# bwittmann/transoar

Measured on AMD Instinct MI355X. Metric: training-step CT volumes/s, 160x160x256 Focused-Decoder, higher is better.
Workload: dtype bf16

## Files before the change

### include/transoar_convgemm.h

```cpp
#ifndef TRANSOAR_CONVGEMM_H
#define TRANSOAR_CONVGEMM_H

#ifdef __cplusplus
extern "C" {
#endif

enum {
  TRANSOAR_CONVGEMM_OK = 0,
  TRANSOAR_CONVGEMM_ERR_NULL = -1,
  TRANSOAR_CONVGEMM_ERR_DIM = -2
};

int transoar_conv3d_igemm(const void* x, const void* wk, const float* bias, void* y, float* y32,
                          int N, int SD, int SH, int SW, int Cin, int Cout,
                          int MD, int MH, int MW, int src_stride,
                          int OD, int OH, int OW, int out_stride, int opd, int oph, int opw,
                          unsigned taps_d, unsigned taps_h, unsigned taps_w, int split, int classes, void* hip_stream);

int transoar_conv3d_finish(const float* y32, const float* bias, void* y, long rows, int cout, int split, void* hip_stream);

int transoar_conv3d_dgrad_s2_halo(const void* dy, const void* wkt, void* dx, int N, int OD, int OH, int OW, int D, int H, int W,
                                  int Cin, int Cout, void* hip_stream);

long transoar_conv3d_wgrad_part_floats(int Cin, int Cout, int chunks, int taps_out);
int transoar_conv3d_wgrad(const void* dy, const void* x, float* part, float* dw, int N, int SD, int SH, int SW, int Cin,
                          int Cout, int MD, int MH, int MW, int src_stride,
                          unsigned taps_d, unsigned taps_h, unsigned taps_w, int chunks, int taps_out, void* hip_stream);

int transoar_linear_wgrad_bias(const void* dy, const void* x, float* part, float* dw, float* bias_part, float* db, int T, int Cin,
                               int Cout, int chunks, void* hip_stream);

int transoar_conv3d_wgrad_ring(const void* dy, const void* x, float* part, float* dw, int N, int SD, int SH, int SW, int Cin,
                               int Cout, int MD, int MH, int MW, int src_stride, int chunks, void* hip_stream);

int transoar_conv3d_pack(const float* w, void* wk, void* wkt, int Cout, int Cin, void* hip_stream);

int transoar_conv3d_pack_many(const void* table, int n_layers, long total_tiles, void* hip_stream);

int transoar_convgemm_abi_version(void);

#ifdef __cplusplus
}
#endif
#endif
```

### transoar_amd/conv_gemm.py

```python
import os

import torch

from . import _native
from ._native import launch, ptr

ABI_VERSION = 3
CL3D = torch.channels_last_3d
lib = _native.bind("convgemm", abi=ABI_VERSION)


def _taps(entries):
    v = len(entries)
    for e, (delta, t) in enumerate(entries):
        v |= ((delta + 1) << (2 + 4 * e)) | (t << (4 + 4 * e))
    return v


TAPS_FWD = _taps([(-1, 0), (0, 1), (1, 2)])
TAPS_DGRAD1 = _taps([(1, 0), (0, 1), (-1, 2)])
TAPS_PARITY = (_taps([(0, 1)]), _taps([(1, 0), (0, 2)]))
TAPS_ONE = _taps([(0, 1)])

SPLIT_BELOW_TILES = 384
DGRAD_S2_HALO = os.environ.get("TRANSOAR_DGRAD_S2_HALO", "1") != "0"
WGRAD_BLOCKS = 512


def pack_fwd(weight):
    co, ci = weight.shape[:2]
    return weight.permute(2, 3, 4, 0, 1).reshape(27, co, ci).to(torch.bfloat16).contiguous()


def pack_dgrad(weight):
    co, ci = weight.shape[:2]
    return weight.permute(2, 3, 4, 1, 0).reshape(27, ci, co).to(torch.bfloat16).contiguous()


def pack_both(weight):
    co, ci = weight.shape[:2]
    if weight.dtype != torch.float32 or not weight.is_contiguous() or not os.environ.get("TRANSOAR_CONV_PACK_HIP"):
        return pack_fwd(weight), pack_dgrad(weight)
    wk = torch.empty((27, co, ci), dtype=torch.bfloat16, device=weight.device)
    wkt = torch.empty((27, ci, co), dtype=torch.bfloat16, device=weight.device)
    launch(lib.transoar_conv3d_pack, weight, weight.data_ptr(), wk.data_ptr(), wkt.data_ptr(), co, ci)
    return wk, wkt


class PackPlan:

    def __init__(self, modules):
        self.modules = list(modules)
        assert self.modules
        dev = self.modules[0].weight.device
        self.buffers, rows, tile = [], [], 0
        for m in self.modules:
            w = m.weight
            assert w.dtype == torch.float32 and w.is_contiguous() and tuple(w.shape[2:]) == (3, 3, 3) and w.device == dev
            co, ci = w.shape[:2]
            wk = torch.empty((27, co, ci), dtype=torch.bfloat16, device=dev)
            wkt = torch.empty((27, ci, co), dtype=torch.bfloat16, device=dev)
            self.buffers.append((wk, wkt))
            rows.append([w.data_ptr(), wk.data_ptr(), wkt.data_ptr(), co | (ci << 32), tile])
            tile += ((co + 31) // 32) * ((ci + 31) // 32)
        self.total_tiles = tile
        self.ptrs = [r[0] for r in rows]
        self.table = torch.tensor(rows, dtype=torch.int64, device=dev)

    def valid(self):
        return all(m.weight.data_ptr() == p for m, p in zip(self.modules, self.ptrs))

    def run(self):
        launch(lib.transoar_conv3d_pack_many, self.table, self.table.data_ptr(), len(self.modules), self.total_tiles)
        for m, packs in zip(self.modules, self.buffers):
            m._packs, m._packs_version = packs, m.weight._version


def _split_for(tiles, k_steps):
    if tiles >= SPLIT_BELOW_TILES:
        return 1
    return max(1, min((SPLIT_BELOW_TILES + tiles - 1) // tiles, k_steps // 4, 16))


def _tiles(rows, cout):
    bn = 64 if cout <= 64 else 128
    return ((rows + 127) // 128) * ((cout + bn - 1) // bn)


def _igemm(x, wk, bias, out, src_dims, cin, cout, m_dims, src_stride, out_dims, out_stride, parity, taps, n, split, classes=0):
    if split > 1:
        rows_out = n * out_dims[0] * out_dims[1] * out_dims[2]
        part = torch.empty((split, rows_out, cout), dtype=torch.float32, device=x.device)
        launch(lib.transoar_conv3d_igemm, x, x.data_ptr(), wk.data_ptr(), None, None, part.data_ptr(), n, *src_dims, cin, cout,
               *m_dims, src_stride, *out_dims, out_stride, *parity, *taps, split, classes)
        launch(lib.transoar_conv3d_finish, x, part.data_ptr(), ptr(bias), out.data_ptr(), rows_out, cout, split)
    else:
        launch(lib.transoar_conv3d_igemm, x, x.data_ptr(), wk.data_ptr(), ptr(bias), out.data_ptr(), None, n, *src_dims, cin, cout,
               *m_dims, src_stride, *out_dims, out_stride, *parity, *taps, 1, classes)


MAX_ROWS = 1 << 21


def _batch_chunks(n, rows_per_sample, what):
    if n * rows_per_sample < MAX_ROWS:
        return [(0, n)]
    per = (MAX_ROWS - 1) // rows_per_sample
    if per < 1:
        raise RuntimeError("%s: one sample has %d rows, the implicit-GEMM kernels address < %d per launch"
                           % (what, rows_per_sample, MAX_ROWS))
    return [(i, min(per, n - i)) for i in range(0, n, per)]


def conv_forward(x, wk, bias, stride, split=None):
    n, ci, d, h, w = x.shape
    co = wk.shape[1]
    od, oh, ow = (d - 1) // stride + 1, (h - 1) // stride + 1, (w - 1) // stride + 1
    chunks = _batch_chunks(n, od * oh * ow, "conv_forward")
    if len(chunks) > 1:
        y = torch.empty((n, co, od, oh, ow), dtype=torch.bfloat16, device=x.device, memory_format=CL3D)
        for i, c in chunks:
            y[i:i + c] = conv_forward(x[i:i + c], wk, bias, stride, split)
        return y
    y = torch.empty((n, co, od, oh, ow), dtype=torch.bfloat16, device=x.device, memory_format=CL3D)
    if split is None:
        split = _split_for(_tiles(n * od * oh * ow, co), (27 * ci + 63) // 64)
    _igemm(x, wk, bias, y, (d, h, w), ci, co, (od, oh, ow), stride, (od, oh, ow), 1, (0, 0, 0), (TAPS_FWD,) * 3, n, split)
    return y


def conv_dgrad(gy, wkt, stride, in_dims, split=None):
    n, co, od, oh, ow = gy.shape
    ci = wkt.shape[1]
    d, h, w = in_dims
    gx = torch.empty((n, ci, d, h, w), dtype=torch.bfloat16, device=gy.device, memory_format=CL3D)
    halo = split is None and stride == 2 and DGRAD_S2_HALO and ci <= 32 and co in (16, 32, 48)
    chunks = [(0, n)] if halo else _batch_chunks(n, d * h * w, "conv_dgrad")
    if len(chunks) > 1:
        for i, c in chunks:
            gx[i:i + c] = conv_dgrad(gy[i:i + c], wkt, stride, in_dims, split)
        return gx
    if stride == 1:
        if split is None:
            split = _split_for(_tiles(n * d * h * w, ci), (27 * co + 63) // 64)
        _igemm(gy, wkt, None, gx, (od, oh, ow), co, ci, (d, h, w), 1, (d, h, w), 1, (0, 0, 0), (TAPS_DGRAD1,) * 3, n, split)
        return gx
    if split is None and DGRAD_S2_HALO and ci <= 32 and co in (16, 32, 48):
        launch(lib.transoar_conv3d_dgrad_s2_halo, gy, gy.data_ptr(), wkt.data_ptr(), gx.data_ptr(), n, od, oh, ow, d, h, w, ci, co)
        return gx
    if split is None:
        split = _split_for(_tiles(n * d * h * w, ci), (8 * co + 63) // 64)
    _igemm(gy, wkt, None, gx, (od, oh, ow), co, ci, (1, 1, 1), 1, (d, h, w), 2, (0, 0, 0), (TAPS_ONE,) * 3, n, split, classes=1)
    return gx


def _wgrad(x2, gy2, geom, taps, taps_out, out_shape):
    n, sd, sh, sw, ci, co, md, mh, mw, stride = geom
    nt = 1
    for t in taps:
        nt *= t & 3
    bt = 64 if (ci <= 64 and co <= 64) else 128
    tiles = nt * ((co + bt - 1) // bt) * ((ci + bt - 1) // bt)
    rows = n * md * mh * mw
    budget = WGRAD_BLOCKS * (2 if (rows >= (1 << 20) or tiles >= 64) else 1)
    chunks = max(1, min(budget // tiles, rows // 1024 if rows >= 1024 else 1))
    part = torch.empty(lib.transoar_conv3d_wgrad_part_floats(ci, co, chunks, taps_out), dtype=torch.float32, device=x2.device)
    dw = torch.empty(out_shape, dtype=torch.float32, device=x2.device)
    launch(lib.transoar_conv3d_wgrad, x2, gy2.data_ptr(), x2.data_ptr(), part.data_ptr(), dw.data_ptr(), n, sd, sh, sw, ci, co,
           md, mh, mw, stride, *taps, chunks, taps_out)
    return dw


WGRAD_RING = os.environ.get("TRANSOAR_WGRAD_RING", "1") != "0"
WGRAD_RING_CHUNKS = 85


def wgrad_ring_supported(ci, co, ow, rows):
    return (WGRAD_RING and ci <= 64 and co <= 64 and max(ci, co) > 32 and ci % 8 == 0 and co % 8 == 0 and ow % 64 == 0
            and rows >= (1 << 18))


def conv_wgrad_ring(x, gy, stride, chunks=None):
    n, ci, d, h, w = x.shape
    co, od, oh, ow = gy.shape[1:]
    chunks = chunks or WGRAD_RING_CHUNKS
    part = torch.empty(lib.transoar_conv3d_wgrad_part_floats(ci, co, chunks, 27), dtype=torch.float32, device=x.device)
    dw = torch.empty((co, ci, 3, 3, 3), dtype=torch.float32, device=x.device)
    launch(lib.transoar_conv3d_wgrad_ring, x, gy.data_ptr(), x.data_ptr(), part.data_ptr(), dw.data_ptr(), n, d, h, w, ci, co,
           od, oh, ow, stride, chunks)
    return dw


def conv_wgrad(x, gy, stride):
    n, ci, d, h, w = x.shape
    co, od, oh, ow = gy.shape[1:]
    if wgrad_ring_supported(ci, co, ow, n * od * oh * ow):
        return conv_wgrad_ring(x, gy, stride)
    chunks = _batch_chunks(n, od * oh * ow, "conv_wgrad")
    if len(chunks) > 1:
        dw = None
        for i, c in chunks:
            part = conv_wgrad(x[i:i + c], gy[i:i + c], stride)
            dw = part if dw is None else dw.add_(part)
        return dw
    return _wgrad(x, gy, (n, d, h, w, ci, co, od, oh, ow, stride), (TAPS_FWD,) * 3, 27, (co, ci, 3, 3, 3))


def linear_wgrad(x, gy):
    t, k = x.shape
    nn_ = gy.shape[1]
    return _wgrad(x, gy, (1, 1, 1, t, k, nn_, 1, 1, t, 1), (TAPS_ONE,) * 3, 1, (nn_, k))


def linear_wgrad_bias_usable(k, n):
    return k % (64 if (k <= 64 and n <= 64) else 128) != 0


def linear_wgrad_bias(x, gy):
    t, k = x.shape
    nn_ = gy.shape[1]
    bt = 64 if (k <= 64 and nn_ <= 64) else 128
    tiles = ((nn_ + bt - 1) // bt) * ((k + bt - 1) // bt)
    budget = WGRAD_BLOCKS * (2 if (t >= (1 << 20) or tiles >= 64) else 1)
    chunks = max(1, min(budget // tiles, t // 1024 if t >= 1024 else 1))
    part = torch.empty(lib.transoar_conv3d_wgrad_part_floats(k, nn_, chunks, 1), dtype=torch.float32, device=x.device)
    bias_part = torch.empty(chunks * nn_, dtype=torch.float32, device=x.device)
    dw = torch.empty((nn_, k), dtype=torch.float32, device=x.device)
    db = torch.empty(nn_, dtype=torch.float32, device=x.device)
    launch(lib.transoar_linear_wgrad_bias, x, gy.data_ptr(), x.data_ptr(), part.data_ptr(), dw.data_ptr(), bias_part.data_ptr(),
           db.data_ptr(), t, k, nn_, chunks)
    return dw, db


def supported(cin, cout, rows):
    return cin % 8 == 0 and cout % 8 == 0 and cin >= 8 and rows < (1 << 21)
```

### transoar_amd/csrc/conv_gemm.hip

```cpp
#include <hip/hip_runtime.h>
#include <stdint.h>

#include "../../include/transoar_convgemm.h"

namespace {

typedef float f32x16 __attribute__((ext_vector_type(16)));
typedef short s16x8 __attribute__((ext_vector_type(8)));
typedef short s16x4 __attribute__((ext_vector_type(4)));
typedef __bf16 bf16x8_t __attribute__((ext_vector_type(8)));
typedef unsigned int u32x4 __attribute__((ext_vector_type(4)));

constexpr int BM = 128, BK = 64;
constexpr int kTile = BM * BK * 2;

__device__ __forceinline__ f32x16 mfma(s16x8 a, s16x8 b, f32x16 c) {
  return __builtin_amdgcn_mfma_f32_32x32x16_bf16(__builtin_bit_cast(bf16x8_t, a), __builtin_bit_cast(bf16x8_t, b), c, 0, 0, 0);
}
__device__ __forceinline__ unsigned short f32_to_bf16(float f) {
  return __builtin_bit_cast(unsigned short, static_cast<__bf16>(f));
}
typedef __attribute__((address_space(3))) void conv_lds_void;
__device__ __forceinline__ void dma16(__amdgpu_buffer_rsrc_t rs, unsigned voff, unsigned dst) {
  unsigned keep;
  asm volatile(
      "s_nop 4\n\t"
      "s_mov_b32 %0, m0\n\t"
      "s_mov_b32 m0, %3\n\t"
      "s_nop 0\n\t"
      "buffer_load_dwordx4 %1, %2, 0 offen lds\n\t"
      "s_mov_b32 m0, %0"
      : "=&s"(keep)
      : "v"(voff), "s"(rs), "s"(dst)
      : "memory");
}
__device__ __forceinline__ void dma_wait() { asm volatile("s_waitcnt vmcnt(0)" ::: "memory"); }
__device__ __forceinline__ void block_barrier() { asm volatile("s_waitcnt lgkmcnt(0)\n\ts_barrier" ::: "memory"); }

__device__ __forceinline__ long xcd_contiguous(long bid, long n) {
  const long per = (n + 7) >> 3;
  const long swz = (bid & 7) * per + (bid >> 3);
  return swz < n ? swz : -1;
}

__device__ __forceinline__ int taps_count(unsigned p) { return p & 3; }
__device__ __forceinline__ int taps_delta(unsigned p, int e) { return static_cast<int>((p >> (2 + 4 * e)) & 3) - 1; }
__device__ __forceinline__ int taps_t(unsigned p, int e) { return (p >> (4 + 4 * e)) & 3; }

struct ConvGeom {
  int N, SD, SH, SW;
  int MD, MH, MW;
  int OD, OH, OW;
  int src_stride, out_stride, opd, oph, opw;
  int Cin, Cout;
};

constexpr int kInvalid = 0x40000000;
constexpr unsigned kTapsParity0 = 1u | (1u << 2) | (1u << 4);
constexpr unsigned kTapsParity1 = 2u | (2u << 2) | (0u << 4) | (1u << 6) | (2u << 8);

template <int TN>
__global__ __launch_bounds__(256, 2) void conv3d_igemm_kernel(
    const unsigned short* __restrict__ X, const unsigned short* __restrict__ Wk, const float* __restrict__ bias,
    unsigned short* __restrict__ Y, float* __restrict__ y32, ConvGeom g, unsigned tp_d, unsigned tp_h, unsigned tp_w,
    int split, long n_tiles, int tiles_n, int classes, unsigned x_bytes, unsigned w_bytes) {
  constexpr int BNT = 64 * TN, NB = BNT / 32;
  __shared__ __attribute__((aligned(16))) unsigned char lds[2][kTile + BNT * BK * 2];
  __shared__ int2 tap_tab[32];
  const int tid = threadIdx.x, lane = tid & 63, wave = tid >> 6;
  const long tile_id = xcd_contiguous(blockIdx.x, n_tiles * split);
  if (tile_id < 0) return;
  const int ks = static_cast<int>(tile_id / n_tiles);
  long t = tile_id - static_cast<long>(ks) * n_tiles;
  if (classes) {
    for (int c = 7; c >= 0; --c) {
      const int pd = (c >> 2) & 1, ph = (c >> 1) & 1, pw = c & 1;
      const int md = (g.OD - pd + 1) >> 1, mh = (g.OH - ph + 1) >> 1, mw = (g.OW - pw + 1) >> 1;
      const long tl = (static_cast<long>(g.N) * md * mh * mw + BM - 1) / BM * tiles_n;
      if (t < tl || c == 0) {
        g.MD = md; g.MH = mh; g.MW = mw; g.opd = pd; g.oph = ph; g.opw = pw;
        tp_d = pd ? kTapsParity1 : kTapsParity0; tp_h = ph ? kTapsParity1 : kTapsParity0; tp_w = pw ? kTapsParity1 : kTapsParity0;
        break;
      }
      t -= tl;
    }
    if (g.MD * g.MH * g.MW == 0) return;
  }
  const int tm = static_cast<int>(t / tiles_n), tn = static_cast<int>(t % tiles_n);
  const int wm = wave >> 1, wn = wave & 1;
  const int m0 = tm * BM, n0 = tn * BNT;
  const int M = g.N * g.MD * g.MH * g.MW;
  const int nd = taps_count(tp_d), nh = taps_count(tp_h), nw = taps_count(tp_w);
  const int ntaps = nd * nh * nw;
  if (tid < 32) {
    int2 e{0, kInvalid};
    if (tid < ntaps) {
      const int ed = tid / (nh * nw), r = tid - ed * nh * nw, eh = r / nw, ew = r - eh * nw;
      e.x = ((taps_delta(tp_d, ed) * g.SH + taps_delta(tp_h, eh)) * g.SW + taps_delta(tp_w, ew)) * g.Cin * 2;
      e.y = ((taps_t(tp_d, ed) * 3 + taps_t(tp_h, eh)) * 3 + taps_t(tp_w, ew)) * g.Cout * g.Cin * 2;
    }
    tap_tab[tid] = e;
  }
  const __amdgpu_buffer_rsrc_t rx = __builtin_amdgcn_make_buffer_rsrc(const_cast<unsigned short*>(X), 0, static_cast<int>(x_bytes), 0x00020000);
  const __amdgpu_buffer_rsrc_t rw = __builtin_amdgcn_make_buffer_rsrc(const_cast<unsigned short*>(Wk), 0, static_cast<int>(w_bytes), 0x00020000);

  const float inv_mw = 1.0f / static_cast<float>(g.MW), inv_mh = 1.0f / static_cast<float>(g.MH), inv_md = 1.0f / static_cast<float>(g.MD);
  auto split_row = [&](int m, int& nb, int& md, int& mh, int& mw) {
    const int r1 = static_cast<int>((static_cast<float>(m) + 0.5f) * inv_mw);
    mw = m - r1 * g.MW;
    const int r2 = static_cast<int>((static_cast<float>(r1) + 0.5f) * inv_mh);
    mh = r1 - r2 * g.MH;
    nb = static_cast<int>((static_cast<float>(r2) + 0.5f) * inv_md);
    md = r2 - nb * g.MD;
  };
  const int s_piece = tid & 7, s_row = tid >> 3;
  unsigned a_base[4], b_base[NB];
  unsigned a_inv[4];
#pragma unroll
  for (int i = 0; i < 4; ++i) {
    const int m = m0 + s_row + 32 * i;
    unsigned ok = 0;
    a_base[i] = 0;
    if (m < M) {
      int nb, md, mh, mw;
      split_row(m, nb, md, mh, mw);
      const int sd = md * g.src_stride, sh = mh * g.src_stride, sw = mw * g.src_stride;
      a_base[i] = static_cast<unsigned>(((nb * g.SD + sd) * g.SH + sh) * g.SW + sw) * static_cast<unsigned>(g.Cin) * 2u;
      unsigned wv = 0, hw = 0;
#pragma unroll
      for (int e = 0; e < 3; ++e)
        wv |= (e < nw && static_cast<unsigned>(sw + taps_delta(tp_w, e)) < static_cast<unsigned>(g.SW)) ? (1u << e) : 0u;
#pragma unroll
      for (int e = 0; e < 3; ++e)
        hw |= (e < nh && static_cast<unsigned>(sh + taps_delta(tp_h, e)) < static_cast<unsigned>(g.SH)) ? (wv << (e * nw)) : 0u;
#pragma unroll
      for (int e = 0; e < 3; ++e)
        ok |= (e < nd && static_cast<unsigned>(sd + taps_delta(tp_d, e)) < static_cast<unsigned>(g.SD)) ? (hw << (e * nh * nw)) : 0u;
    }
    a_inv[i] = ~ok;
  }
#pragma unroll
  for (int i = 0; i < NB; ++i) {
    const int n = n0 + s_row + 32 * i;
    b_base[i] = n < g.Cout ? static_cast<unsigned>(n) * static_cast<unsigned>(g.Cin) * 2u : static_cast<unsigned>(kInvalid);
  }
  __syncthreads();

  const int PT = g.Cin >> 3;
  const int pieces = ntaps * PT;
  const int KT = (pieces + 7) >> 3;
  const int kt_per = (KT + split - 1) / split;
  const int kt0 = ks * kt_per, kt1 = min(KT, kt0 + kt_per);
  const float inv_pt = 1.0f / static_cast<float>(PT);

// ... 296 lines not shown
        }
      }
      if (ci >= g.Cin) continue;
#pragma unroll
      for (int r = 0; r < 16; ++r) {
        const int co = co0 + wm * 32 * TW + a * 32 + (r & 3) + 8 * (r >> 2) + 4 * kg;
        if (co < g.Cout) dst[static_cast<long>(co) * g.Cin + ci] = acc[a][b][r];
      }
    }
}

constexpr int kReducePairs = 128;
__global__ __launch_bounds__(256) void conv3d_wgrad_reduce_kernel(const float* __restrict__ part, float* __restrict__ dw, int chunks,
                                                                  int slabs, long coci) {
  __shared__ __attribute__((aligned(16))) float sh[kReducePairs * 27];
  const long e0 = static_cast<long>(blockIdx.x) * kReducePairs;
  const int quads = kReducePairs / 4;
  const int work = quads * slabs;
  if (work < 256) {
    const int P = 256 / work;
    const int sub = threadIdx.x / work, idx = threadIdx.x - sub * work;
    const int tap = idx / quads, q = idx - tap * quads;
    float4 v{0.f, 0.f, 0.f, 0.f};
    if (sub < P && e0 + 4 * q < coci) {
      const float* src = part + static_cast<long>(tap) * coci + e0 + 4 * q;
      const long step = static_cast<long>(slabs) * coci;
      int k = sub;
      for (; k + 3 * P < chunks; k += 4 * P) {
        const float4 a = *reinterpret_cast<const float4*>(src + (k + 0 * P) * step), b = *reinterpret_cast<const float4*>(src + (k + 1 * P) * step);
        const float4 c = *reinterpret_cast<const float4*>(src + (k + 2 * P) * step), d = *reinterpret_cast<const float4*>(src + (k + 3 * P) * step);
        v.x += (a.x + b.x) + (c.x + d.x); v.y += (a.y + b.y) + (c.y + d.y);
        v.z += (a.z + b.z) + (c.z + d.z); v.w += (a.w + b.w) + (c.w + d.w);
      }
      for (; k < chunks; k += P) {
        const float4 a = *reinterpret_cast<const float4*>(src + k * step);
        v.x += a.x; v.y += a.y; v.z += a.z; v.w += a.w;
      }
    }
    float4* turn = reinterpret_cast<float4*>(sh);
    if (sub < P) turn[sub * work + idx] = v;
    __syncthreads();
    if (sub == 0) {
      for (int g2 = 1; g2 < P; ++g2) {
        const float4 o = turn[g2 * work + idx];
        v.x += o.x; v.y += o.y; v.z += o.z; v.w += o.w;
      }
    }
    __syncthreads();
    if (sub == 0) {
      sh[(4 * q + 0) * slabs + tap] = v.x;
      sh[(4 * q + 1) * slabs + tap] = v.y;
      sh[(4 * q + 2) * slabs + tap] = v.z;
      sh[(4 * q + 3) * slabs + tap] = v.w;
    }
  } else {
  for (int idx = threadIdx.x; idx < quads * slabs; idx += 256) {
    const int tap = idx / quads, q = idx - tap * quads;
    float4 v{0.f, 0.f, 0.f, 0.f};
    if (e0 + 4 * q < coci) {
      const float* src = part + static_cast<long>(tap) * coci + e0 + 4 * q;
      const long step = static_cast<long>(slabs) * coci;
      int k = 0;
      for (; k + 4 <= chunks; k += 4) {
        const float4 a = *reinterpret_cast<const float4*>(src + (k + 0) * step), b = *reinterpret_cast<const float4*>(src + (k + 1) * step);
        const float4 c = *reinterpret_cast<const float4*>(src + (k + 2) * step), d = *reinterpret_cast<const float4*>(src + (k + 3) * step);
        v.x += (a.x + b.x) + (c.x + d.x); v.y += (a.y + b.y) + (c.y + d.y);
        v.z += (a.z + b.z) + (c.z + d.z); v.w += (a.w + b.w) + (c.w + d.w);
      }
      for (; k < chunks; ++k) {
        const float4 a = *reinterpret_cast<const float4*>(src + k * step);
        v.x += a.x; v.y += a.y; v.z += a.z; v.w += a.w;
      }
    }
    sh[(4 * q + 0) * slabs + tap] = v.x;
    sh[(4 * q + 1) * slabs + tap] = v.y;
    sh[(4 * q + 2) * slabs + tap] = v.z;
    sh[(4 * q + 3) * slabs + tap] = v.w;
  }
  }
  __syncthreads();
  const long total = coci * slabs, base = e0 * slabs;
  for (int idx = threadIdx.x; idx < quads * slabs; idx += 256)
    if (base + 4 * idx < total) *reinterpret_cast<float4*>(dw + base + 4 * idx) = *reinterpret_cast<const float4*>(&sh[4 * idx]);
}

__global__ __launch_bounds__(256) void conv3d_pack_kernel(const float* __restrict__ w, unsigned short* __restrict__ wk,
                                                          unsigned short* __restrict__ wkt, int co_n, int ci_n) {
  __shared__ unsigned short sh[27][32][33];
  const int tiles_ci = (ci_n + 31) / 32;
  const int co0 = (blockIdx.x / tiles_ci) * 32, ci0 = (blockIdx.x % tiles_ci) * 32;
  for (int idx = threadIdx.x; idx < 32 * 32 * 27; idx += 256) {
    const int col = idx % (32 * 27), a = idx / (32 * 27);
    const int b = col / 27, tap = col - b * 27;
    const int co = co0 + a, ci = ci0 + b;
    float v = 0.f;
    if (co < co_n && ci < ci_n) v = w[(static_cast<long>(co) * ci_n + ci) * 27 + tap];
    sh[tap][a][b] = f32_to_bf16(v);
  }
  __syncthreads();
  for (int idx = threadIdx.x; idx < 27 * 32 * 32; idx += 256) {
    const int x = idx & 31, y = (idx >> 5) & 31, tap = idx >> 10;
    if (co0 + y < co_n && ci0 + x < ci_n) wk[(static_cast<long>(tap) * co_n + co0 + y) * ci_n + ci0 + x] = sh[tap][y][x];
    if (wkt != nullptr && ci0 + y < ci_n && co0 + x < co_n) wkt[(static_cast<long>(tap) * ci_n + ci0 + y) * co_n + co0 + x] = sh[tap][x][y];
  }
}

struct PackEntry {
  const float* w;
  unsigned short* wk;
  unsigned short* wkt;
  long co_ci;
  long tile_begin;
};
__global__ __launch_bounds__(256) void conv3d_pack_many_kernel(const PackEntry* __restrict__ table, int n_layers) {
  constexpr int P = 34;
  __shared__ __attribute__((aligned(16))) unsigned short sh[27][32][P];
  int l = 0;
  while (l + 1 < n_layers && static_cast<long>(blockIdx.x) >= table[l + 1].tile_begin) ++l;
  const PackEntry e = table[l];
  const int co_n = static_cast<int>(e.co_ci & 0xffffffffL), ci_n = static_cast<int>(e.co_ci >> 32);
  const int tile = static_cast<int>(blockIdx.x - e.tile_begin);
  const int tiles_ci = (ci_n + 31) / 32;
  const int co0 = (tile / tiles_ci) * 32, ci0 = (tile % tiles_ci) * 32;
  const int ci_valid = min(32, ci_n - ci0);
  for (int idx = threadIdx.x; idx < 32 * 216; idx += 256) {
    const int a = idx / 216, f = idx - a * 216;
    float4 v{0.f, 0.f, 0.f, 0.f};
    if (co0 + a < co_n && 4 * f < ci_valid * 27)
      v = *reinterpret_cast<const float4*>(e.w + (static_cast<long>(co0 + a) * ci_n + ci0) * 27 + 4 * f);
    const float vv[4] = {v.x, v.y, v.z, v.w};
#pragma unroll
    for (int j = 0; j < 4; ++j) {
      const int p = 4 * f + j, b = p / 27, tap = p - b * 27;
      sh[tap][a][b] = f32_to_bf16(vv[j]);
    }
  }
  __syncthreads();
  for (int idx = threadIdx.x; idx < 27 * 32 * 4; idx += 256) {
    const int x8 = idx & 3, y = (idx >> 2) & 31, tap = idx >> 7;
    if (co0 + y < co_n && ci0 + 8 * x8 < ci_n) {
      const unsigned* src = reinterpret_cast<const unsigned*>(&sh[tap][y][8 * x8]);
      *reinterpret_cast<u32x4*>(e.wk + (static_cast<long>(tap) * co_n + co0 + y) * ci_n + ci0 + 8 * x8) = u32x4{src[0], src[1], src[2], src[3]};
    }
    if (e.wkt != nullptr && ci0 + y < ci_n && co0 + 8 * x8 < co_n) {
      unsigned r[4];
#pragma unroll
      for (int j = 0; j < 4; ++j)
        r[j] = static_cast<unsigned>(sh[tap][8 * x8 + 2 * j][y]) | (static_cast<unsigned>(sh[tap][8 * x8 + 2 * j + 1][y]) << 16);
      *reinterpret_cast<u32x4*>(e.wkt + (static_cast<long>(tap) * ci_n + ci0 + y) * co_n + co0 + 8 * x8) = u32x4{r[0], r[1], r[2], r[3]};
    }
  }
}

#include "conv_dgrad_s2.hpp"
#include "conv_wgrad_ring.hpp"

int check_geom(const ConvGeom& g) {
  if (g.N <= 0 || g.SD <= 0 || g.SH <= 0 || g.SW <= 0 || g.MD <= 0 || g.MH <= 0 || g.MW <= 0 || g.OD <= 0 || g.OH <= 0 || g.OW <= 0 ||
      g.Cin <= 0 || g.Cout <= 0 || (g.Cin & 7) || (g.Cout & 7) || g.src_stride < 1 || g.src_stride > 2 || g.out_stride < 1 || g.out_stride > 2)
    return TRANSOAR_CONVGEMM_ERR_DIM;
  const long src = static_cast<long>(g.N) * g.SD * g.SH * g.SW * g.Cin * 2, out = static_cast<long>(g.N) * g.OD * g.OH * g.OW * g.Cout * 2;
  const long rows = static_cast<long>(g.N) * g.MD * g.MH * g.MW;
  if (src >= 0x7ffffff0L || out >= 0x7ffffff0L * 2 || rows >= (1L << 31) || rows * g.Cout * 2 >= 0x7ffffff0L * 2 || 27L * g.Cout * g.Cin * 2 >= 0x3ffffff0L)
    return TRANSOAR_CONVGEMM_ERR_DIM;
  return 0;
}
bool taps_ok(unsigned p) { return (p & 3) >= 1 && (p & 3) <= 3; }

}

extern "C" int transoar_conv3d_igemm(const void* x, const void* wk, const float* bias, void* y, float* y32, int N, int SD,
                                     int SH, int SW, int Cin, int Cout, int MD, int MH, int MW, int src_stride, int OD, int OH,
                                     int OW, int out_stride, int opd, int oph, int opw, unsigned taps_d, unsigned taps_h,
                                     unsigned taps_w, int split, int classes, void* hip_stream) {
  if (!x || !wk || (!y && !y32)) return TRANSOAR_CONVGEMM_ERR_NULL;
  if (classes) {
    MD = (OD + 1) / 2; MH = (OH + 1) / 2; MW = (OW + 1) / 2;
    src_stride = 1; out_stride = 2; opd = oph = opw = 0;
    taps_d = taps_h = taps_w = kTapsParity1;
  }
  const ConvGeom g{N, SD, SH, SW, MD, MH, MW, OD, OH, OW, src_stride, out_stride, opd, oph, opw, Cin, Cout};
  const int rc = check_geom(g);
  if (rc) return rc;
  if (!taps_ok(taps_d) || !taps_ok(taps_h) || !taps_ok(taps_w) || split < 1 || (split > 1 && !y32)) return TRANSOAR_CONVGEMM_ERR_DIM;
  if (static_cast<long>(N) * MD * MH * MW >= (1L << 21)) return TRANSOAR_CONVGEMM_ERR_DIM;
  hipStream_t st = static_cast<hipStream_t>(hip_stream);
  const bool narrow = Cout <= 64;
  const int bn = narrow ? 64 : 128;
  const int tiles_n = (Cout + bn - 1) / bn;
  long n_tiles = 0;
  if (classes) {
    for (int c = 0; c < 8; ++c) {
      const long md = (OD - ((c >> 2) & 1) + 1) / 2, mh = (OH - ((c >> 1) & 1) + 1) / 2, mw = (OW - (c & 1) + 1) / 2;
      n_tiles += (N * md * mh * mw + BM - 1) / BM * tiles_n;
    }
  } else {
    n_tiles = (static_cast<long>(N) * MD * MH * MW + BM - 1) / BM * tiles_n;
  }
  const long blocks = ((n_tiles * split + 7) / 8) * 8;
  const unsigned xb = static_cast<unsigned>(static_cast<long>(N) * SD * SH * SW * Cin * 2), wb = static_cast<unsigned>(27L * Cout * Cin * 2);
  if (narrow)
    hipLaunchKernelGGL(conv3d_igemm_kernel<1>, dim3(static_cast<unsigned>(blocks)), dim3(256), 0, st, static_cast<const unsigned short*>(x),
                       static_cast<const unsigned short*>(wk), bias, static_cast<unsigned short*>(y), y32, g, taps_d, taps_h, taps_w,
                       split, n_tiles, tiles_n, classes, xb, wb);
  else
    hipLaunchKernelGGL(conv3d_igemm_kernel<2>, dim3(static_cast<unsigned>(blocks)), dim3(256), 0, st, static_cast<const unsigned short*>(x),
                       static_cast<const unsigned short*>(wk), bias, static_cast<unsigned short*>(y), y32, g, taps_d, taps_h, taps_w,
                       split, n_tiles, tiles_n, classes, xb, wb);
  return static_cast<int>(hipGetLastError());
}

extern "C" int transoar_conv3d_dgrad_s2_halo(const void* dy, const void* wkt, void* dx, int N, int OD, int OH, int OW, int D, int H, int W,
                                            int Cin, int Cout, void* hip_stream) {
  if (!dy || !wkt || !dx) return TRANSOAR_CONVGEMM_ERR_NULL;
  if (N <= 0 || OD <= 0 || OH <= 0 || OW <= 0 || Cin <= 0 || Cin > 32 || (Cin & 7) || (Cout != 16 && Cout != 32 && Cout != 48))
    return TRANSOAR_CONVGEMM_ERR_DIM;
  if ((D != 2 * OD && D != 2 * OD - 1) || (H != 2 * OH && H != 2 * OH - 1) || (W != 2 * OW && W != 2 * OW - 1)) return TRANSOAR_CONVGEMM_ERR_DIM;
  const long dy_bytes = static_cast<long>(N) * OD * OH * OW * Cout * 2;
  if (dy_bytes >= 0x7ffffff0L || (4L * H + 8) * W * Cin * 2 >= 0x7ffffff0L) return TRANSOAR_CONVGEMM_ERR_DIM;
  const int td = (OD + kDs2TD - 1) / kDs2TD, th = (OH + kDs2TH - 1) / kDs2TH, tw = (OW + kDs2TW - 1) / kDs2TW;
  const long n_tiles = static_cast<long>(N) * td * th * tw;
  static int resident[3] = {0, 0, 0};
  const int ki = Cout / 16 - 1;
  if (!resident[ki]) {
    int per_cu = 0, dev = 0;
    hipDeviceProp_t prop;
    const void* fn = ki == 0 ? reinterpret_cast<const void*>(conv3d_dgrad_s2_halo_kernel<1>)
                   : ki == 1 ? reinterpret_cast<const void*>(conv3d_dgrad_s2_halo_kernel<2>) : reinterpret_cast<const void*>(conv3d_dgrad_s2_halo_kernel<3>);
    if (hipGetDevice(&dev) != hipSuccess || hipGetDeviceProperties(&prop, dev) != hipSuccess ||
        hipOccupancyMaxActiveBlocksPerMultiprocessor(&per_cu, fn, 256, 0) != hipSuccess || per_cu < 1)
      return TRANSOAR_CONVGEMM_ERR_DIM;
    resident[ki] = per_cu * prop.multiProcessorCount;
  }
  const unsigned blocks = static_cast<unsigned>(n_tiles < resident[ki] ? n_tiles : resident[ki]);
  hipStream_t st = static_cast<hipStream_t>(hip_stream);
#define TRANSOAR_DS2_LAUNCH(KS)                                                                                                     \
  hipLaunchKernelGGL(conv3d_dgrad_s2_halo_kernel<KS>, dim3(blocks), dim3(256), 0, st, static_cast<const unsigned short*>(dy),       \
                     static_cast<const unsigned short*>(wkt), static_cast<unsigned short*>(dx), N, OD, OH, OW, D, H, W, Cin, td, th, tw, \
                     static_cast<unsigned>(dy_bytes))
  if (Cout == 16) TRANSOAR_DS2_LAUNCH(1);
  else if (Cout == 32) TRANSOAR_DS2_LAUNCH(2);
  else TRANSOAR_DS2_LAUNCH(3);
#undef TRANSOAR_DS2_LAUNCH
  return static_cast<int>(hipGetLastError());
}

extern "C" int transoar_conv3d_finish(const float* y32, const float* bias, void* y, long rows, int cout, int split, void* hip_stream) {
  if (!y32 || !y) return TRANSOAR_CONVGEMM_ERR_NULL;
  if (rows <= 0 || cout <= 0 || (cout & 7) || split < 1) return TRANSOAR_CONVGEMM_ERR_DIM;
  const long n8 = rows * cout / 8;
  hipLaunchKernelGGL(conv3d_finish_kernel, dim3(static_cast<unsigned>((n8 + 255) / 256)), dim3(256), 0, static_cast<hipStream_t>(hip_stream),
                     y32, bias, static_cast<unsigned short*>(y), n8, cout, split);
  return static_cast<int>(hipGetLastError());
}

extern "C" long transoar_conv3d_wgrad_part_floats(int Cin, int Cout, int chunks, int taps_out) { return static_cast<long>(taps_out) * Cin * Cout * chunks; }

static int wgrad_launch(const void* dy, const void* x, float* part, float* dw, int N, int SD, int SH, int SW, int Cin,
                        int Cout, int MD, int MH, int MW, int src_stride, unsigned taps_d, unsigned taps_h,
                        unsigned taps_w, int chunks, int taps_out, float* bias_part, float* db, void* hip_stream) {
  if (!dy || !x || !part || !dw) return TRANSOAR_CONVGEMM_ERR_NULL;
  const ConvGeom g{N, SD, SH, SW, MD, MH, MW, MD, MH, MW, src_stride, 1, 0, 0, 0, Cin, Cout};
  const int rc = check_geom(g);
  if (rc) return rc;
  if (!taps_ok(taps_d) || !taps_ok(taps_h) || !taps_ok(taps_w) || chunks < 1 || (taps_out != 1 && taps_out != 27)) return TRANSOAR_CONVGEMM_ERR_DIM;
  const long M = static_cast<long>(N) * MD * MH * MW;
  if (M >= (1L << 21)) return TRANSOAR_CONVGEMM_ERR_DIM;
  const int max_chunks = chunks;
  if (chunks > M) chunks = static_cast<int>(M);
  const int rows_per_chunk = static_cast<int>(((M + chunks - 1) / chunks + WK - 1) / WK * WK);
  chunks = static_cast<int>((M + rows_per_chunk - 1) / rows_per_chunk);
  if (chunks > max_chunks) return TRANSOAR_CONVGEMM_ERR_DIM;
  const int ntaps = static_cast<int>((taps_d & 3) * (taps_h & 3) * (taps_w & 3));
  if (taps_out == 1 && ntaps != 1) return TRANSOAR_CONVGEMM_ERR_DIM;
  hipStream_t st = static_cast<hipStream_t>(hip_stream);
  const bool small = Cin <= 64 && Cout <= 64;
  const int bt = small ? 64 : 128;
  const int tiles_co = (Cout + bt - 1) / bt, tiles_ci = (Cin + bt - 1) / bt;
  const long blocks = (static_cast<long>(chunks) * tiles_ci * tiles_co * ntaps + 7) / 8 * 8;
  if (blocks >= (1L << 31)) return TRANSOAR_CONVGEMM_ERR_DIM;
  const unsigned dyb = static_cast<unsigned>(M * Cout * 2), xb = static_cast<unsigned>(static_cast<long>(N) * SD * SH * SW * Cin * 2);
  if (small)
    hipLaunchKernelGGL(conv3d_wgrad_kernel<1>, dim3(static_cast<unsigned>(blocks)), dim3(256), 0, st, static_cast<const unsigned short*>(dy),
                       static_cast<const unsigned short*>(x), part, g, taps_d, taps_h, taps_w, chunks, rows_per_chunk, tiles_co, tiles_ci, taps_out, dyb, xb, bias_part);
  else
    hipLaunchKernelGGL(conv3d_wgrad_kernel<2>, dim3(static_cast<unsigned>(blocks)), dim3(256), 0, st, static_cast<const unsigned short*>(dy),
                       static_cast<const unsigned short*>(x), part, g, taps_d, taps_h, taps_w, chunks, rows_per_chunk, tiles_co, tiles_ci, taps_out, dyb, xb, bias_part);
  const long coci = static_cast<long>(Cout) * Cin;
  hipLaunchKernelGGL(conv3d_wgrad_reduce_kernel, dim3(static_cast<unsigned>((coci + kReducePairs - 1) / kReducePairs)), dim3(256), 0, st, part, dw, chunks, taps_out, coci);
  if (bias_part != nullptr)
    hipLaunchKernelGGL(conv3d_wgrad_reduce_kernel, dim3(static_cast<unsigned>((Cout + kReducePairs - 1) / kReducePairs)), dim3(256), 0, st, bias_part, db, chunks, 1,
                       static_cast<long>(Cout));
  return static_cast<int>(hipGetLastError());
}

extern "C" int transoar_conv3d_wgrad(const void* dy, const void* x, float* part, float* dw, int N, int SD, int SH, int SW, int Cin,
                                     int Cout, int MD, int MH, int MW, int src_stride, unsigned taps_d, unsigned taps_h,
                                     unsigned taps_w, int chunks, int taps_out, void* hip_stream) {
  return wgrad_launch(dy, x, part, dw, N, SD, SH, SW, Cin, Cout, MD, MH, MW, src_stride, taps_d, taps_h, taps_w, chunks, taps_out, nullptr, nullptr,
                      hip_stream);
}

extern "C" int transoar_linear_wgrad_bias(const void* dy, const void* x, float* part, float* dw, float* bias_part, float* db, int T,
                                          int Cin, int Cout, int chunks, void* hip_stream) {
  if (!bias_part || !db) return TRANSOAR_CONVGEMM_ERR_NULL;
  const int bt = (Cin <= 64 && Cout <= 64) ? 64 : 128;
  if (Cin % bt == 0) return TRANSOAR_CONVGEMM_ERR_DIM;
  constexpr unsigned kOneTap = 1u | (1u << 2) | (1u << 4);
  return wgrad_launch(dy, x, part, dw, 1, 1, 1, T, Cin, Cout, 1, 1, T, 1, kOneTap, kOneTap, kOneTap, chunks, 1, bias_part, db, hip_stream);
}

extern "C" int transoar_conv3d_wgrad_ring(const void* dy, const void* x, float* part, float* dw, int N, int SD, int SH, int SW, int Cin,
                                          int Cout, int MD, int MH, int MW, int src_stride, int chunks, void* hip_stream) {
  if (!dy || !x || !part || !dw) return TRANSOAR_CONVGEMM_ERR_NULL;
  if (N <= 0 || SD <= 0 || SH <= 0 || SW <= 0 || MD <= 0 || MH <= 0 || MW <= 0 || Cin <= 0 || Cout <= 0 || (Cin & 7) || (Cout & 7) ||
      Cin > 64 || Cout > 64 || (MW & 63) || chunks < 1 || (src_stride != 1 && src_stride != 2))
    return TRANSOAR_CONVGEMM_ERR_DIM;
  if (MD != (SD - 1) / src_stride + 1 || MH != (SH - 1) / src_stride + 1 || MW != (SW - 1) / src_stride + 1) return TRANSOAR_CONVGEMM_ERR_DIM;
  const int tiles_co = (Cout + 31) / 32, tiles_ci = (Cin + 31) / 32;
  if (tiles_co * tiles_ci < 2) return TRANSOAR_CONVGEMM_ERR_DIM;
  const long columns = static_cast<long>(N) * MD * (MW / 64);
  int h_chunks = 1;
  while (columns * h_chunks < 4L * chunks && (MH + h_chunks) / (h_chunks + 1) >= 8) ++h_chunks;
  const int h_chunk = (MH + h_chunks - 1) / h_chunks;
  h_chunks = (MH + h_chunk - 1) / h_chunk;
  hipStream_t st = static_cast<hipStream_t>(hip_stream);
  const dim3 grid(static_cast<unsigned>(chunks * 3));
  auto dys = static_cast<const unsigned short*>(dy);
  auto xs = static_cast<const unsigned short*>(x);
#define TRANSOAR_RING_LAUNCH(S_, CIT_)                                                                                                    \
  hipLaunchKernelGGL((conv3d_wgrad_ring_kernel<S_, CIT_>), grid, dim3(512), 0, st, dys, xs, part, N, SD, SH, SW, MD, MH, MW, Cin, Cout, tiles_co, \
                     tiles_ci, h_chunks, h_chunk)
  if (src_stride == 1) { if (tiles_ci == 1) TRANSOAR_RING_LAUNCH(1, 1); else TRANSOAR_RING_LAUNCH(1, 2); }
  else { if (tiles_ci == 1) TRANSOAR_RING_LAUNCH(2, 1); else TRANSOAR_RING_LAUNCH(2, 2); }
#undef TRANSOAR_RING_LAUNCH
  const long coci = static_cast<long>(Cout) * Cin;
  hipLaunchKernelGGL(conv3d_wgrad_reduce_kernel, dim3(static_cast<unsigned>((coci + kReducePairs - 1) / kReducePairs)), dim3(256), 0, st, part, dw, chunks, 27, coci);
  return static_cast<int>(hipGetLastError());
}

extern "C" int transoar_conv3d_pack(const float* w, void* wk, void* wkt, int Cout, int Cin, void* hip_stream) {
  if (!w || !wk) return TRANSOAR_CONVGEMM_ERR_NULL;
  if (Cout <= 0 || Cin <= 0) return TRANSOAR_CONVGEMM_ERR_DIM;
  const int blocks = ((Cout + 31) / 32) * ((Cin + 31) / 32);
  hipLaunchKernelGGL(conv3d_pack_kernel, dim3(blocks), dim3(256), 0, static_cast<hipStream_t>(hip_stream), w,
                     static_cast<unsigned short*>(wk), static_cast<unsigned short*>(wkt), Cout, Cin);
  return static_cast<int>(hipGetLastError());
}

extern "C" int transoar_conv3d_pack_many(const void* table, int n_layers, long total_tiles, void* hip_stream) {
  if (!table) return TRANSOAR_CONVGEMM_ERR_NULL;
  if (n_layers <= 0 || total_tiles <= 0 || total_tiles >= (1L << 31)) return TRANSOAR_CONVGEMM_ERR_DIM;
  hipLaunchKernelGGL(conv3d_pack_many_kernel, dim3(static_cast<unsigned>(total_tiles)), dim3(256), 0, static_cast<hipStream_t>(hip_stream),
                     static_cast<const PackEntry*>(table), n_layers);
  return static_cast<int>(hipGetLastError());
}

extern "C" int transoar_convgemm_abi_version(void) { return 3; }
```

Measured before the change: 64.77.

## Add line-tiled implicit-GEMM conv kernel reusing W-halo rows across taps

Adds a specialised implicit-GEMM kernel for stride-1, unsplit 3x3x3 convolutions whose output tile covers whole W lines. It loads each line once with a one-voxel halo into LDS and reuses it for all three W taps, which cuts global A traffic and DMA count roughly threefold. The K loop interleaves next-stage DMA issue with MFMA groups. The dispatcher routes matching forward and stride-1 dgrad calls to it, and new Python route helpers expose the eligibility test. The cost is extra complexity, different LDS usage and occupancy, and geometry restrictions.

```diff
diff --git a/include/transoar_convgemm.h b/include/transoar_convgemm.h
--- a/include/transoar_convgemm.h
+++ b/include/transoar_convgemm.h
@@ -16,6 +16,11 @@
                           int MD, int MH, int MW, int src_stride,
                           int OD, int OH, int OW, int out_stride, int opd, int oph, int opw,
                           unsigned taps_d, unsigned taps_h, unsigned taps_w, int split, int classes, void* hip_stream);
+
+int transoar_conv3d_igemm_route(int N, int SD, int SH, int SW, int Cin, int Cout,
+                                int MD, int MH, int MW, int src_stride,
+                                int OD, int OH, int OW, int out_stride, int opd, int oph, int opw,
+                                unsigned taps_d, unsigned taps_h, unsigned taps_w, int split, int classes);
 
 int transoar_conv3d_finish(const float* y32, const float* bias, void* y, long rows, int cout, int split, void* hip_stream);
 
diff --git a/transoar_amd/conv_gemm.py b/transoar_amd/conv_gemm.py
--- a/transoar_amd/conv_gemm.py
+++ b/transoar_amd/conv_gemm.py
@@ -154,6 +154,21 @@
     return gx
 
 
+def forward_route(n, ci, co, d, h, w, stride, split=None):
+    od, oh, ow = (d - 1) // stride + 1, (h - 1) // stride + 1, (w - 1) // stride + 1
+    if split is None:
+        split = _split_for(_tiles(n * od * oh * ow, co), (27 * ci + 63) // 64)
+    return lib.transoar_conv3d_igemm_route(n, d, h, w, ci, co, od, oh, ow, stride, od, oh, ow, 1, 0, 0, 0, *(TAPS_FWD,) * 3, split, 0)
+
+
+def dgrad_route(n, ci, co, d, h, w, stride, split=None):
+    if stride != 1:
+        return 0
+    if split is None:
+        split = _split_for(_tiles(n * d * h * w, ci), (27 * co + 63) // 64)
+    return lib.transoar_conv3d_igemm_route(n, d, h, w, co, ci, d, h, w, 1, d, h, w, 1, 0, 0, 0, *(TAPS_DGRAD1,) * 3, split, 0)
+
+
 def _wgrad(x2, gy2, geom, taps, taps_out, out_shape):
     n, sd, sh, sw, ci, co, md, mh, mw, stride = geom
     nt = 1
diff --git a/transoar_amd/csrc/conv_gemm.hip b/transoar_amd/csrc/conv_gemm.hip
--- a/transoar_amd/csrc/conv_gemm.hip
+++ b/transoar_amd/csrc/conv_gemm.hip
@@ -1,5 +1,7 @@
 #include <hip/hip_runtime.h>
 #include <stdint.h>
+
+#include <type_traits>
 
 #include "../../include/transoar_convgemm.h"
 
@@ -602,6 +604,7 @@
   }
 }
 
+#include "conv_igemm_line.hpp"
 #include "conv_dgrad_s2.hpp"
 #include "conv_wgrad_ring.hpp"
 
@@ -649,6 +652,15 @@
   }
   const long blocks = ((n_tiles * split + 7) / 8) * 8;
   const unsigned xb = static_cast<unsigned>(static_cast<long>(N) * SD * SH * SW * Cin * 2), wb = static_cast<unsigned>(27L * Cout * Cin * 2);
+  if (y && !y32 && line_kernel_fits(g, taps_d, taps_h, taps_w, split, classes)) {
+    if (narrow)
+      hipLaunchKernelGGL(conv3d_igemm_line_kernel<1>, dim3(static_cast<unsigned>(blocks)), dim3(256), 0, st, static_cast<const unsigned short*>(x),
+                         static_cast<const unsigned short*>(wk), bias, static_cast<unsigned short*>(y), g, taps_d, taps_h, taps_w, n_tiles, tiles_n, xb, wb);
+    else
+      hipLaunchKernelGGL(conv3d_igemm_line_kernel<2>, dim3(static_cast<unsigned>(blocks)), dim3(256), 0, st, static_cast<const unsigned short*>(x),
+                         static_cast<const unsigned short*>(wk), bias, static_cast<unsigned short*>(y), g, taps_d, taps_h, taps_w, n_tiles, tiles_n, xb, wb);
+    return static_cast<int>(hipGetLastError());
+  }
   if (narrow)
     hipLaunchKernelGGL(conv3d_igemm_kernel<1>, dim3(static_cast<unsigned>(blocks)), dim3(256), 0, st, static_cast<const unsigned short*>(x),
                        static_cast<const unsigned short*>(wk), bias, static_cast<unsigned short*>(y), y32, g, taps_d, taps_h, taps_w,
@@ -658,6 +670,13 @@
                        static_cast<const unsigned short*>(wk), bias, static_cast<unsigned short*>(y), y32, g, taps_d, taps_h, taps_w,
                        split, n_tiles, tiles_n, classes, xb, wb);
   return static_cast<int>(hipGetLastError());
+}
+
+extern "C" int transoar_conv3d_igemm_route(int N, int SD, int SH, int SW, int Cin, int Cout, int MD, int MH, int MW, int src_stride,
+                                           int OD, int OH, int OW, int out_stride, int opd, int oph, int opw, unsigned taps_d,
+                                           unsigned taps_h, unsigned taps_w, int split, int classes) {
+  const ConvGeom g{N, SD, SH, SW, MD, MH, MW, OD, OH, OW, src_stride, out_stride, opd, oph, opw, Cin, Cout};
+  return line_kernel_fits(g, taps_d, taps_h, taps_w, split, classes) ? 1 : 0;
 }
 
 extern "C" int transoar_conv3d_dgrad_s2_halo(const void* dy, const void* wkt, void* dx, int N, int OD, int OH, int OW, int D, int H, int W,
diff --git a/transoar_amd/csrc/conv_igemm_line.hpp b/transoar_amd/csrc/conv_igemm_line.hpp
--- /dev/null
+++ b/transoar_amd/csrc/conv_igemm_line.hpp
@@ -0,0 +1,273 @@
+#ifndef LINE_INTERLEAVE
+#define LINE_INTERLEAVE 1
+#endif
+#ifndef LINE_TRIM
+#define LINE_TRIM 1
+#endif
+constexpr int LK = 32;
+constexpr int kLineRows = 192;
+constexpr int kLineA = kLineRows * LK * 2;
+
+template <int TN>
+__global__ __launch_bounds__(256, 2) void conv3d_igemm_line_kernel(
+    const unsigned short* __restrict__ X, const unsigned short* __restrict__ Wk, const float* __restrict__ bias,
+    unsigned short* __restrict__ Y, ConvGeom g, unsigned tp_d, unsigned tp_h, unsigned tp_w, long n_tiles, int tiles_n,
+    unsigned x_bytes, unsigned w_bytes) {
+  constexpr int BNT = 64 * TN;
+  constexpr int NBI = 3 * TN;
+  constexpr unsigned kStage = kLineA + 3 * BNT * LK * 2;
+  __shared__ __attribute__((aligned(16))) unsigned char lds[2][kStage];
+  __shared__ int2 ent_tab[16];
+  const int tid = threadIdx.x, lane = tid & 63, wave = tid >> 6;
+  const long t = xcd_contiguous(blockIdx.x, n_tiles);
+  if (t < 0) return;
+  const int tm = static_cast<int>(t / tiles_n), tn = static_cast<int>(t % tiles_n);
+  const int wm = wave >> 1, wn = wave & 1;
+  const int m0 = tm * BM, n0 = tn * BNT;
+  const int M = g.N * g.MD * g.MH * g.MW;
+  const int LW = min(g.MW, BM), SLW = LW + 2;
+  const int lines = BM / LW;
+  const int lw_shift = 31 - __builtin_clz(static_cast<unsigned>(LW));
+  if (tid < 16) {
+    int2 e{0, kInvalid};
+    if (tid < 9) {
+      const int ed = tid / 3, eh = tid - ed * 3;
+      e.x = (taps_delta(tp_d, ed) * g.SH + taps_delta(tp_h, eh)) * g.SW * g.Cin * 2;
+      e.y = (taps_t(tp_d, ed) * 3 + taps_t(tp_h, eh)) * 3 * g.Cout * g.Cin * 2;
+    }
+    ent_tab[tid] = e;
+  }
+  const __amdgpu_buffer_rsrc_t rx = __builtin_amdgcn_make_buffer_rsrc(const_cast<unsigned short*>(X), 0, static_cast<int>(x_bytes), 0x00020000);
+  const __amdgpu_buffer_rsrc_t rw = __builtin_amdgcn_make_buffer_rsrc(const_cast<unsigned short*>(Wk), 0, static_cast<int>(w_bytes), 0x00020000);
+
+  const int s_row = wave * 16 + (lane >> 2);
+  const int l_piece = (lane & 3) ^ ((lane >> 4) & 3);
+  const float inv_mw = 1.0f / static_cast<float>(g.MW), inv_mh = 1.0f / static_cast<float>(g.MH), inv_md = 1.0f / static_cast<float>(g.MD);
+  const float inv_slw = 1.0f / static_cast<float>(SLW);
+  unsigned a_base[3], a_inv[3], b_base[NBI];
+#pragma unroll
+  for (int i = 0; i < 3; ++i) {
+    const int s = s_row + 64 * i;
+    const int l = static_cast<int>((static_cast<float>(s) + 0.5f) * inv_slw), j = s - l * SLW;
+    const int ml = m0 + l * LW;
+    unsigned ok = 0;
+    a_base[i] = 0;
+    if (l < lines && ml < M) {
+      const int r1 = static_cast<int>((static_cast<float>(ml) + 0.5f) * inv_mw), w0 = ml - r1 * g.MW;
+      const int r2 = static_cast<int>((static_cast<float>(r1) + 0.5f) * inv_mh), mh = r1 - r2 * g.MH;
+      const int nb = static_cast<int>((static_cast<float>(r2) + 0.5f) * inv_md), md = r2 - nb * g.MD;
+      const int sw = w0 + j - 1;
+      a_base[i] = static_cast<unsigned>(((nb * g.SD + md) * g.SH + mh) * g.SW + sw) * static_cast<unsigned>(g.Cin) * 2u;
+      if (static_cast<unsigned>(sw) < static_cast<unsigned>(g.SW)) {
+        unsigned hv = 0;
+#pragma unroll
+        for (int e = 0; e < 3; ++e)
+          hv |= static_cast<unsigned>(mh + taps_delta(tp_h, e)) < static_cast<unsigned>(g.SH) ? (1u << e) : 0u;
+#pragma unroll
+        for (int e = 0; e < 3; ++e)
+          ok |= static_cast<unsigned>(md + taps_delta(tp_d, e)) < static_cast<unsigned>(g.SD) ? (hv << (3 * e)) : 0u;
+      }
+    }
+    a_inv[i] = ~ok;
+  }
+#pragma unroll
+  for (int i = 0; i < NBI; ++i) {
+    const int rb = s_row + 64 * i;
+    const int ew = rb / BNT, n = n0 + rb - ew * BNT;
+    b_base[i] = n < g.Cout ? static_cast<unsigned>(taps_t(tp_w, ew) * g.Cout + n) * static_cast<unsigned>(g.Cin) * 2u
+                           : static_cast<unsigned>(kInvalid);
+  }
+  __syncthreads();
+
+  const int PT = g.Cin >> 3;
+  const int KT = (9 * PT + 3) >> 2;
+  const float inv_pt = 1.0f / static_cast<float>(PT);
+  const unsigned lds0 = static_cast<unsigned>(reinterpret_cast<size_t>((conv_lds_void*)&lds[0][0]));
+  const unsigned dst0 = __builtin_amdgcn_readfirstlane(lds0 + static_cast<unsigned>(wave) * 1024u);
+  constexpr int NDMA = 3 + NBI;
+  unsigned d_voff[NDMA], d_base = 0;
+#if defined(LINE_PROBE_A) || defined(LINE_PROBE_B)
+  bool d_probe_skip = false;
+#endif
+#if LINE_TRIM
+  const int a_chunks = (lines * SLW + 15) >> 4;
+  const int wave_u = __builtin_amdgcn_readfirstlane(wave);
+#endif
+  auto dma_prepare = [&](int kt, int stage) {
+    const int j = kt * 4 + l_piece;
+    const int e = min(static_cast<int>((static_cast<float>(j) + 0.5f) * inv_pt), 15);
+    const int c8 = j - __mul24(e, PT);
+    const int2 tt = ent_tab[e];
+    const unsigned src = static_cast<unsigned>(tt.x + c8 * 16), wof = static_cast<unsigned>(tt.y + c8 * 16);
+    d_base = dst0 + static_cast<unsigned>(stage) * kStage;
+#pragma unroll
+    for (int i = 0; i < 3; ++i) d_voff[i] = (a_base[i] + src) | (((a_inv[i] >> e) & 1u) << 31);
+#pragma unroll
+    for (int i = 0; i < NBI; ++i) d_voff[3 + i] = b_base[i] + wof;
+  };
+  auto dma_issue = [&](int idx) {
+#if defined(LINE_PROBE_A)
+    if (idx < 3 && d_probe_skip) return;
+#endif
+#if defined(LINE_PROBE_B)
+    if (idx >= 3 && d_probe_skip) return;
+#endif
+#if LINE_TRIM
+    if (idx < 3 && idx * 4 + wave_u >= a_chunks) return;
+#endif
+    if (idx < 3) dma16(rx, d_voff[idx], d_base + idx * 4096u);
+    else dma16(rw, d_voff[idx], d_base + kLineA + (idx - 3) * 4096u);
+  };
+  auto dma_step = [&](int kt, int stage) {
+    dma_prepare(kt, stage);
+#pragma unroll
+    for (int i = 0; i < NDMA; ++i) dma_issue(i);
+  };
+
+  f32x16 acc[TN][2];
+#pragma unroll
+  for (int a = 0; a < TN; ++a)
+#pragma unroll
+    for (int b = 0; b < 2; ++b)
+#pragma unroll
+      for (int i = 0; i < 16; ++i) acc[a][b][i] = 0.f;
+  const int fr = lane & 31, kg = lane >> 5;
+  int fa_off[2][2][3], fb_off[2][TN];
+#pragma unroll
+  for (int k2 = 0; k2 < 2; ++k2) {
+    const int piece = 2 * k2 + kg;
+#pragma unroll
+    for (int i = 0; i < 2; ++i) {
+      const int rm = wm * 64 + i * 32 + fr;
+      const int s1 = (rm >> lw_shift) * SLW + (rm & (LW - 1)) + 1;
+#pragma unroll
+      for (int ew = 0; ew < 3; ++ew) {
+        const int s = s1 + taps_delta(tp_w, ew);
+        fa_off[k2][i][ew] = s * (LK * 2) + ((piece ^ ((s >> 2) & 3)) << 4);
+      }
+    }
+#pragma unroll
+    for (int i = 0; i < TN; ++i) {
+      const int rn = wn * 32 * TN + i * 32 + fr;
+      fb_off[k2][i] = rn * (LK * 2) + ((piece ^ ((rn >> 2) & 3)) << 4);
+    }
+  }
+  auto compute = [&](int stage, auto fetch) {
+    const unsigned char* ta = lds[stage];
+    const unsigned char* tb = lds[stage] + kLineA;
+#pragma unroll
+    for (int k2 = 0; k2 < 2; ++k2) {
+#pragma unroll
+      for (int ew = 0; ew < 3; ++ew) {
+        s16x8 fa[2], fb[TN];
+#pragma unroll
+        for (int i = 0; i < 2; ++i) fa[i] = *reinterpret_cast<const s16x8*>(ta + fa_off[k2][i][ew]);
+#pragma unroll
+        for (int i = 0; i < TN; ++i) fb[i] = *reinterpret_cast<const s16x8*>(tb + fb_off[k2][i] + ew * (BNT * LK * 2));
+#pragma unroll
+        for (int a = 0; a < TN; ++a)
+#pragma unroll
+          for (int b = 0; b < 2; ++b) acc[a][b] = mfma(fb[a], fa[b], acc[a][b]);
+#if LINE_INTERLEAVE
+        if constexpr (decltype(fetch)::value) {
+          const int grp = k2 * 3 + ew;
+          dma_issue(grp);
+          if (grp + 6 < NDMA) dma_issue(grp + 6);
+          __builtin_amdgcn_sched_barrier(0);
+        }
+#endif
+      }
+    }
+  };
+  constexpr std::true_type kFetch{};
+  constexpr std::false_type kNoFetch{};
+  dma_step(0, 0);
+#if defined(LINE_PROBE_A) || defined(LINE_PROBE_B)
+  d_probe_skip = true;
+#endif
+  dma_wait();
+  block_barrier();
+  int kt = 0;
+#if LINE_INTERLEAVE
+  for (; kt + 2 < KT; kt += 2) {
+    dma_prepare(kt + 1, 1);
+    compute(0, kFetch);
+    dma_wait();
+    block_barrier();
+    dma_prepare(kt + 2, 0);
+    compute(1, kFetch);
+    dma_wait();
+    block_barrier();
+  }
+  if (kt + 2 == KT) {
+    dma_prepare(kt + 1, 1);
+    compute(0, kFetch);
+    dma_wait();
+    block_barrier();
+    compute(1, kNoFetch);
+    block_barrier();
+    kt += 2;
+  }
+#else
+  for (; kt + 2 <= KT; kt += 2) {
+    dma_step(kt + 1, 1);
+    compute(0, kNoFetch);
+    dma_wait();
+    block_barrier();
+    if (kt + 2 < KT) dma_step(kt + 2, 0);
+    compute(1, kNoFetch);
+    dma_wait();
+    block_barrier();
+  }
+#endif
+  if (kt < KT) {
+    compute(0, kNoFetch);
+    block_barrier();
+  }
+
+  constexpr int PITCH = 32 * TN * 2 + 16;
+  unsigned char* stage = &lds[0][0] + wave * (64 * PITCH);
+#pragma unroll
+  for (int b = 0; b < 2; ++b)
+#pragma unroll
+    for (int a = 0; a < TN; ++a)
+#pragma unroll
+      for (int q = 0; q < 4; ++q) {
+        const int nl = a * 32 + 8 * q + 4 * kg;
+        const int n = n0 + wn * 32 * TN + nl;
+        float4 bv{0.f, 0.f, 0.f, 0.f};
+        if (bias != nullptr && n < g.Cout) bv = *reinterpret_cast<const float4*>(bias + n);
+        const float bq4[4] = {bv.x, bv.y, bv.z, bv.w};
+        unsigned short h[4];
+#pragma unroll
+        for (int e = 0; e < 4; ++e) h[e] = f32_to_bf16(acc[a][b][4 * q + e] + bq4[e]);
+        *reinterpret_cast<uint2*>(stage + (b * 32 + fr) * PITCH + nl * 2) =
+            uint2{static_cast<unsigned>(h[0]) | (static_cast<unsigned>(h[1]) << 16), static_cast<unsigned>(h[2]) | (static_cast<unsigned>(h[3]) << 16)};
+      }
+  constexpr int PP = 4 * TN, RP = 64 / PP;
+  const int piece = lane % PP, r0 = lane / PP;
+#pragma unroll
+  for (int it = 0; it < PP; ++it) {
+    const int row = it * RP + r0;
+    const int m = m0 + wm * 64 + row, n = n0 + wn * 32 * TN + piece * 8;
+    if (m < M && n < g.Cout) {
+      const u32x4 v = *reinterpret_cast<const u32x4*>(stage + row * PITCH + piece * 16);
+      *reinterpret_cast<u32x4*>(Y + static_cast<long>(m) * g.Cout + n) = v;
+    }
+  }
+}
+
+inline bool taps_are_unit_shifts(unsigned p) {
+  if ((p & 3) != 3) return false;
+  unsigned seen = 0;
+  for (int e = 0; e < 3; ++e) seen |= 1u << ((p >> (2 + 4 * e)) & 3);
+  return seen == 7u;
+}
+inline bool line_kernel_fits(const ConvGeom& g, unsigned tp_d, unsigned tp_h, unsigned tp_w, int split, int classes) {
+  if (classes != 0 || split != 1 || g.src_stride != 1 || g.out_stride != 1) return false;
+  if (!taps_are_unit_shifts(tp_d) || !taps_are_unit_shifts(tp_h) || !taps_are_unit_shifts(tp_w)) return false;
+  if (g.OD != g.MD || g.OH != g.MH || g.OW != g.MW || g.opd || g.oph || g.opw) return false;
+  if (g.SD != g.MD || g.SH != g.MH || g.SW != g.MW) return false;
+  if (g.MW < 16 || (BM % g.MW != 0 && g.MW % BM != 0)) return false;
+  return (g.Cin & 7) == 0;
+}
```

Result: no change. 65.23, median of 6 (+0.7%).
